# ch-andrei/VTAMIQ

Hardware: AMD Instinct MI355X
Metric: image-pairs/sec ViT-B/16 P=500 patches, 1->8 MI355X; % bf16 MFMA roofline (higher is better)
Workload: dtype f16

## Files before the change

### vtamiq_amd/csrc/cls_tail.hip

```cpp
#include <mutex>

#include "dev_common.h"
#include "kernels.h"

namespace vtq {
namespace {

template <int V4>
__global__ __launch_bounds__(256) void rows_ln_kernel(const float* __restrict__ src, int64_t stride, const float* __restrict__ w,
                                                      const float* __restrict__ b, float* __restrict__ ln, float* __restrict__ copy,
                                                      int rows, PlaneOut po, const int* __restrict__ vl_row0) {
    constexpr int H = 256 * V4;
    const int lane = threadIdx.x & 63;
    const int r = blockIdx.x * 4 + (threadIdx.x >> 6);
    if (r >= rows) return;
    const float4* xr = (const float4*)(src + (vl_row0 ? (int64_t)vl_row0[r] * H : r * stride));
    float4 v[V4];
    float s = 0.f;
#pragma unroll
    for (int i = 0; i < V4; ++i) {
        v[i] = xr[i * 64 + lane];
        if (copy) ((float4*)(copy + (int64_t)r * H))[i * 64 + lane] = v[i];
        s += (v[i].x + v[i].y) + (v[i].z + v[i].w);
    }
    const float mean = wave_sum(s) * (1.0f / H);
    float q = 0.f;
#pragma unroll
    for (int i = 0; i < V4; ++i) {
        v[i].x -= mean; v[i].y -= mean; v[i].z -= mean; v[i].w -= mean;
        q += (v[i].x * v[i].x + v[i].y * v[i].y) + (v[i].z * v[i].z + v[i].w * v[i].w);
    }
    const float rstd = 1.0f / sqrtf(wave_sum(q) * (1.0f / H) + 1e-6f);
#pragma unroll
    for (int i = 0; i < V4; ++i) {
        const float4 w4 = ((const float4*)w)[i * 64 + lane], b4 = ((const float4*)b)[i * 64 + lane];
        float4 y = {v[i].x * rstd * w4.x + b4.x, v[i].y * rstd * w4.y + b4.y, v[i].z * rstd * w4.z + b4.z, v[i].w * rstd * w4.w + b4.w};
        ((float4*)(ln + (int64_t)r * H))[i * 64 + lane] = y;
        plane_store4(po, r, (i * 64 + lane) * 4, y.x, y.y, y.z, y.w);
    }
}

constexpr int kFoldChunk = 64;
constexpr int kFoldSub = 32;
constexpr int kFoldPad = 16;

template <typename T, int WPL>
__global__ __launch_bounds__(1024) void cls_key_fold_kernel(const float* __restrict__ q, const T* __restrict__ wk, int64_t w_plane, int ldw,
                                                            float* __restrict__ u, int R, int H) {
    typedef typename Vec<T>::x4 tx4;
    __shared__ float qs[4][64];
    __shared__ __attribute__((aligned(16))) float red[3][4][1024];
    const int head = blockIdx.x, nh = gridDim.x, r0 = blockIdx.y * 4;
    const int ct = H >> 2, g = threadIdx.x / ct, c = 4 * (threadIdx.x - g * ct);
    const T* wr = wk + ((int64_t)head * 64 + g * 16) * ldw + c;
    tx4 wh[16], wl[16];
#pragma unroll
    for (int i = 0; i < 16; ++i) {
        wh[i] = *(const tx4*)(wr + (int64_t)i * ldw);
        if constexpr (WPL == 2) wl[i] = *(const tx4*)(wr + (int64_t)i * ldw + w_plane);
    }
    if (threadIdx.x < 256) {
        const int rr = threadIdx.x >> 6, d = threadIdx.x & 63;
        qs[rr][d] = (r0 + rr < R) ? q[(int64_t)(r0 + rr) * H + head * 64 + d] : 0.f;
    }
    __syncthreads();
    float acc[4][4];
#pragma unroll
    for (int rr = 0; rr < 4; ++rr)
#pragma unroll
        for (int e = 0; e < 4; ++e) acc[rr][e] = 0.f;
#pragma unroll
    for (int i = 0; i < 16; ++i) {
        float w[4];
#pragma unroll
        for (int e = 0; e < 4; ++e) {
            w[e] = (float)wh[i][e];
            if constexpr (WPL == 2) w[e] += (float)wl[i][e];
        }
#pragma unroll
        for (int rr = 0; rr < 4; ++rr) {
            const float qd = qs[rr][g * 16 + i];
#pragma unroll
            for (int e = 0; e < 4; ++e) acc[rr][e] = fmaf(qd, w[e], acc[rr][e]);
        }
    }
    if (g > 0) {
#pragma unroll
        for (int rr = 0; rr < 4; ++rr) *(float4*)&red[g - 1][rr][c] = float4{acc[rr][0], acc[rr][1], acc[rr][2], acc[rr][3]};
    }
    __syncthreads();
    if (g > 0) return;
#pragma unroll
    for (int rr = 0; rr < 4; ++rr) {
#pragma unroll
        for (int k = 0; k < 3; ++k) {
            const float4 o = *(const float4*)&red[k][rr][c];
            acc[rr][0] += o.x; acc[rr][1] += o.y; acc[rr][2] += o.z; acc[rr][3] += o.w;
        }
        if (r0 + rr < R) *(float4*)(u + ((int64_t)(r0 + rr) * nh + head) * H + c) = float4{acc[rr][0], acc[rr][1], acc[rr][2], acc[rr][3]};
    }
}

template <int V4>
__global__ __launch_bounds__(512) void cls_fold_attention_kernel(const float* __restrict__ x, int64_t seq_stride, const float* __restrict__ lw,
                                                                 const float* __restrict__ lb, const float* __restrict__ u,
                                                                 float* __restrict__ part, int S, int nh, int q_log2, VarSeq vl) {
    constexpr int H = 256 * V4, LD = H + kFoldPad, NG = 4 * V4, NB = 2 * V4;
    extern __shared__ __attribute__((aligned(16))) float fold_smem[];
    float* rows = fold_smem;
    float (*scp)[kFoldSub][16] = (float (*)[kFoldSub][16])(rows + kFoldSub * LD);
    float (*pr)[16] = (float (*)[16])(rows + kFoldSub * LD + 4 * kFoldSub * 16);
    float (*pp)[16] = (float (*)[16])(rows + kFoldSub * LD + 5 * kFoldSub * 16);
    float* run = rows + kFoldSub * LD + 6 * kFoldSub * 16;
    const int tid = threadIdx.x, lane = tid & 63, fr = lane & 15, fq = lane >> 4;
    const int wave = __builtin_amdgcn_readfirstlane(tid >> 6);
    const int chunk = blockIdx.x, seq = blockIdx.y, c0 = chunk * kFoldChunk;
    if (vl.len) {
        S = vl.len[seq];
        if (c0 >= S) return;
    }
    const float* xs = x + (vl.row0 ? (int64_t)vl.row0[seq] * H : (int64_t)seq * seq_stride);
    const int rb = wave & 1, kbase = (wave >> 1) * (H / 4);
    float4 uf[NG];
    {
        const float* ur = u + ((int64_t)seq * nh + (fr < nh ? fr : nh - 1)) * H + kbase + 4 * fq;
#pragma unroll
        for (int j = 0; j < NG; ++j) uf[j] = *(const float4*)(ur + 16 * j);
    }
    float4 v[4][V4];
    auto load_rows = [&](int sub) {
#pragma unroll
        for (int i = 0; i < 4; ++i) {
            const int srow = c0 + sub * kFoldSub + wave * 4 + i;
            if (srow < S) {
                const float4* xr = (const float4*)(xs + (int64_t)srow * H);
#pragma unroll
                for (int k = 0; k < V4; ++k) v[i][k] = xr[k * 64 + lane];
            } else {
#pragma unroll
                for (int k = 0; k < V4; ++k) v[i][k] = float4{0.f, 0.f, 0.f, 0.f};
            }
        }
    };
    f32x4 acc[NB];
#pragma unroll
    for (int b = 0; b < NB; ++b) acc[b] = f32x4{0.f, 0.f, 0.f, 0.f};
    f32x4 accl = {0.f, 0.f, 0.f, 0.f};
    if (tid < 16) run[tid] = -INFINITY;
    const int left = S - c0;
    const int nsub = left >= kFoldChunk ? kFoldChunk / kFoldSub : (left + kFoldSub - 1) / kFoldSub;
    load_rows(0);
    for (int sub = 0; sub < nsub; ++sub) {
        const int s0 = c0 + sub * kFoldSub;
        float4 w4[V4], b4[V4];
#pragma unroll
        for (int k = 0; k < V4; ++k) { w4[k] = ((const float4*)lw)[k * 64 + lane]; b4[k] = ((const float4*)lb)[k * 64 + lane]; }
#pragma unroll
        for (int i = 0; i < 4; ++i) {
            const int row = wave * 4 + i;
            const bool live = s0 + row < S;
            float s = 0.f;
#pragma unroll
            for (int k = 0; k < V4; ++k) s += (v[i][k].x + v[i][k].y) + (v[i][k].z + v[i][k].w);
            const float mean = wave_sum(s) * (1.0f / H);
            float qq = 0.f;
#pragma unroll
            for (int k = 0; k < V4; ++k) {
                v[i][k].x -= mean; v[i][k].y -= mean; v[i][k].z -= mean; v[i][k].w -= mean;
                qq += (v[i][k].x * v[i][k].x + v[i][k].y * v[i][k].y) + (v[i][k].z * v[i][k].z + v[i][k].w * v[i][k].w);
            }
            const float rstd = 1.0f / sqrtf(wave_sum(qq) * (1.0f / H) + 1e-6f);
#pragma unroll
            for (int k = 0; k < V4; ++k) {
                float4 y = {v[i][k].x * rstd * w4[k].x + b4[k].x, v[i][k].y * rstd * w4[k].y + b4[k].y, v[i][k].z * rstd * w4[k].z + b4[k].z,
                            v[i][k].w * rstd * w4[k].w + b4[k].w};
                if (!live) y = float4{0.f, 0.f, 0.f, 0.f};
                *(float4*)(rows + row * LD + (k * 64 + lane) * 4) = y;
            }
        }
        __syncthreads();
        if (sub + 1 < nsub) load_rows(sub + 1);
        {
            f32x4 sa = {0.f, 0.f, 0.f, 0.f}, sb = {0.f, 0.f, 0.f, 0.f};
            const float* ar = rows + (rb * 16 + fr) * LD + kbase + 4 * fq;
#pragma unroll
            for (int j = 0; j < NG; ++j) {
                const float4 a = *(const float4*)(ar + 16 * j);
                sa = __builtin_amdgcn_mfma_f32_16x16x4f32(a.x, uf[j].x, sa, 0, 0, 0);
                sb = __builtin_amdgcn_mfma_f32_16x16x4f32(a.y, uf[j].y, sb, 0, 0, 0);
                sa = __builtin_amdgcn_mfma_f32_16x16x4f32(a.z, uf[j].z, sa, 0, 0, 0);
                sb = __builtin_amdgcn_mfma_f32_16x16x4f32(a.w, uf[j].w, sb, 0, 0, 0);
            }
#pragma unroll
            for (int e = 0; e < 4; ++e) scp[wave >> 1][rb * 16 + 4 * fq + e][fr] = sa[e] + sb[e];
        }
        __syncthreads();
        const int row = tid >> 4, h = tid & 15;
        {
            float sc = (scp[0][row][h] + scp[1][row][h]) + (scp[2][row][h] + scp[3][row][h]);
            if (!q_log2) sc *= 0.125f;
            if (s0 + row >= S || h >= nh) sc = -INFINITY;
            pr[row][h] = sc;
        }
        __syncthreads();
        const float m_old = run[(sub & 1) * 16 + h];
        float mx = m_old;
#pragma unroll 8
        for (int r = 0; r < kFoldSub; ++r) mx = fmaxf(mx, pr[r][h]);
        {
            const float d = pr[row][h] - mx;
            pp[row][h] = h < nh ? (q_log2 ? exp2f(d) : expf(d)) : 0.f;
            if (tid < 16) {
                const float dm = m_old - mx;
                run[((sub + 1) & 1) * 16 + h] = mx;
                run[32 + h] = h < nh ? (q_log2 ? exp2f(dm) : expf(dm)) : 1.f;
            }
        }
        __syncthreads();
        {
            if (sub > 0) {
                const float4 al = *(const float4*)(run + 32 + 4 * fq);
#pragma unroll
                for (int b = 0; b < NB; ++b) { acc[b][0] *= al.x; acc[b][1] *= al.y; acc[b][2] *= al.z; acc[b][3] *= al.w; }
                accl[0] *= al.x; accl[1] *= al.y; accl[2] *= al.z; accl[3] *= al.w;
            }
            float pa[kFoldSub / 4];
#pragma unroll
            for (int s = 0; s < kFoldSub / 4; ++s) pa[s] = pp[4 * s + fq][fr];
#pragma unroll
            for (int s = 0; s < kFoldSub / 4; ++s) {
                const float* br = rows + (4 * s + fq) * LD + 16 * wave + fr;
#pragma unroll
                for (int b = 0; b < NB; ++b) acc[b] = __builtin_amdgcn_mfma_f32_16x16x4f32(pa[s], br[128 * b], acc[b], 0, 0, 0);
                if (wave == 0) accl = __builtin_amdgcn_mfma_f32_16x16x4f32(pa[s], 1.0f, accl, 0, 0, 0);
            }
        }
        __syncthreads();
    }
    float* pz = part + ((int64_t)seq * gridDim.x + chunk) * nh * (H + 2);
#pragma unroll
    for (int b = 0; b < NB; ++b)
#pragma unroll
        for (int e = 0; e < 4; ++e)
            if (4 * fq + e < nh) pz[(4 * fq + e) * H + 16 * wave + 128 * b + fr] = acc[b][e];
    if (tid < nh) pz[nh * H + 2 * tid] = run[(nsub & 1) * 16 + tid];
    if (wave == 0 && fr == 0) {
#pragma unroll
        for (int e = 0; e < 4; ++e)
            if (4 * fq + e < nh) pz[nh * H + 2 * (4 * fq + e) + 1] = accl[e];
    }
}

__global__ __launch_bounds__(256) void cls_fold_combine_kernel(const float* __restrict__ part, int nchunks, int H, PlaneOut po, int q_log2,
                                                               const int* __restrict__ vl_len) {
    const int head = blockIdx.x, nh = gridDim.x, seq = blockIdx.y, c4 = 4 * threadIdx.x;
    if (c4 >= H) return;
    const int64_t ps = (int64_t)nh * (H + 2);
    const float* pb = part + (int64_t)seq * nchunks * ps;
    if (vl_len) nchunks = (vl_len[seq] + kFoldChunk - 1) / kFoldChunk;
    const float* ml = pb + (int64_t)nh * H + 2 * head;
    float mx = -INFINITY;
    for (int c0 = 0; c0 < nchunks; c0 += 8) {
        float mv[8];
#pragma unroll
        for (int i = 0; i < 8; ++i) mv[i] = ml[(c0 + i < nchunks ? c0 + i : nchunks - 1) * ps];
#pragma unroll
        for (int i = 0; i < 8; ++i)
            if (c0 + i < nchunks) mx = fmaxf(mx, mv[i]);
    }
    float l = 0.f, z[4] = {0.f, 0.f, 0.f, 0.f};
    for (int c0 = 0; c0 < nchunks; c0 += 4) {
        float mv[4], lv[4];
        float4 zc[4];
#pragma unroll
        for (int i = 0; i < 4; ++i) {
            const int64_t o = (c0 + i < nchunks ? c0 + i : nchunks - 1) * ps;
            mv[i] = ml[o]; lv[i] = ml[o + 1];
            zc[i] = *(const float4*)(pb + o + (int64_t)head * H + c4);
        }
#pragma unroll
        for (int i = 0; i < 4; ++i) {
            if (c0 + i >= nchunks) break;
            const float d = mv[i] - mx;
            const float w = q_log2 ? exp2f(d) : expf(d);
            l = fmaf(w, lv[i], l);
            z[0] = fmaf(w, zc[i].x, z[0]); z[1] = fmaf(w, zc[i].y, z[1]); z[2] = fmaf(w, zc[i].z, z[2]); z[3] = fmaf(w, zc[i].w, z[3]);
        }
    }
    const float inv = 1.0f / l;
    plane_store4(po, seq, head * H + c4, z[0] * inv, z[1] * inv, z[2] * inv, z[3] * inv);
}

}

hipError_t launch_rows_ln(const float* src, int64_t stride, const float* w, const float* b, float* ln, float* copy, int rows, int H,
                          PlaneOut po, hipStream_t s, const int* vl_row0) {
    const dim3 g((rows + 3) / 4), blk(256);
    if (H == 768) hipLaunchKernelGGL(rows_ln_kernel<3>, g, blk, 0, s, src, stride, w, b, ln, copy, rows, po, vl_row0);
    else if (H == 1024) hipLaunchKernelGGL(rows_ln_kernel<4>, g, blk, 0, s, src, stride, w, b, ln, copy, rows, po, vl_row0);
    else return hipErrorInvalidValue;
    return hipGetLastError();
}

int cls_fold_chunk_rows() { return kFoldChunk; }

namespace {
template <int V4>
hipError_t launch_fold_attention(const float* x, int64_t seq_stride, const float* lw, const float* lb, const float* u, float* part, int nseq,
                                 int S, int nh, int q_log2, hipStream_t s, VarSeq vl) {
    constexpr int lds = (kFoldSub * (256 * V4 + kFoldPad) + 6 * kFoldSub * 16 + 48) * 4;
    {
        static std::mutex mu;
        static bool configured[64] = {false};
        int dev = 0;
        hipError_t e = hipGetDevice(&dev);
        if (e != hipSuccess) return e;
        std::lock_guard<std::mutex> lk(mu);
        if (dev < 0 || dev >= 64) return hipErrorInvalidDevice;
        if (!configured[dev]) {
            e = hipFuncSetAttribute((const void*)cls_fold_attention_kernel<V4>, hipFuncAttributeMaxDynamicSharedMemorySize, lds);
            if (e != hipSuccess) return e;
            configured[dev] = true;
        }
    }
    hipLaunchKernelGGL((cls_fold_attention_kernel<V4>), dim3((S + kFoldChunk - 1) / kFoldChunk, nseq), dim3(512), lds, s, x, seq_stride, lw, lb, u,
                       part, S, nh, q_log2, vl);
    return hipGetLastError();
}
}

hipError_t launch_cls_fold(const float* q, const void* wk, int64_t w_plane, int ldw, int f16_, int wplanes, const float* x, int64_t seq_stride,
                           const float* lw, const float* lb, float* u, float* part, int nseq, int S, int H, PlaneOut zo, hipStream_t s,
                           bool q_log2, VarSeq vl) {
    if ((vl.row0 != nullptr) != (vl.len != nullptr)) return hipErrorInvalidValue;
    if (nseq < 1 || S < 1 || (H != 768 && H != 1024) || ldw < H || ldw % 4 || (wplanes != 1 && wplanes != 2) || seq_stride % 4 || !zo.p || zo.ld < (H / 64) * H)
        return hipErrorInvalidValue;
    const int nh = H / 64, nchunks = (S + kFoldChunk - 1) / kFoldChunk;
    const dim3 gk(nh, (nseq + 3) / 4), blk(256);
#define VTQ_KF(TT, NP) hipLaunchKernelGGL((cls_key_fold_kernel<TT, NP>), gk, dim3(H), 0, s, q, (const TT*)wk, w_plane, ldw, u, nseq, H)
    if (!f16_) { if (wplanes == 1) VTQ_KF(bf16, 1); else VTQ_KF(bf16, 2); }
    else { if (wplanes == 1) VTQ_KF(f16, 1); else VTQ_KF(f16, 2); }
#undef VTQ_KF
    hipError_t e = hipGetLastError();
    if (e != hipSuccess) return e;
    e = H == 768 ? launch_fold_attention<3>(x, seq_stride, lw, lb, u, part, nseq, S, nh, q_log2 ? 1 : 0, s, vl)
                 : launch_fold_attention<4>(x, seq_stride, lw, lb, u, part, nseq, S, nh, q_log2 ? 1 : 0, s, vl);
    if (e != hipSuccess) return e;
    hipLaunchKernelGGL(cls_fold_combine_kernel, dim3(nh, nseq), blk, 0, s, (const float*)part, nchunks, H, zo, q_log2 ? 1 : 0, vl.len);
    return hipGetLastError();
}

}
```

Measured before the change: 2153.

## Batch several fold chunks per workgroup, swizzle LDS rows, use permlane max reduction

The CLS fold-attention kernel now has each workgroup process cpw consecutive 64-row chunks, with cpw chosen so about 256 workgroups launch in total. Partial outputs are still written per chunk, and the next tile's rows are prefetched across chunk boundaries. The LDS row layout is XOR-swizzled to reduce bank conflicts on the MFMA operand reads. The per-row score max now uses permlane16/32 swap reductions plus a small per-wave buffer instead of a 32-iteration LDS scan. The trade-off is fewer workgroups and less parallelism for small batches. The final load is clamped instead of branched, so it reads dummy rows.

```diff
diff --git a/vtamiq_amd/csrc/cls_tail.hip b/vtamiq_amd/csrc/cls_tail.hip
--- a/vtamiq_amd/csrc/cls_tail.hip
+++ b/vtamiq_amd/csrc/cls_tail.hip
@@ -1,3 +1,4 @@
+#include <algorithm>
 #include <mutex>
 
 #include "dev_common.h"
@@ -43,6 +44,23 @@
 constexpr int kFoldChunk = 64;
 constexpr int kFoldSub = 32;
 constexpr int kFoldPad = 16;
+constexpr int kFoldGroupWgs = 256;
+
+template <int M>
+__device__ __forceinline__ float fold_max_xor(float v) {
+    uint32_t a = __builtin_bit_cast(uint32_t, v), b = a;
+    asm volatile("" : "+v"(b));
+    uint32_t s0, s1;
+    if constexpr (M == 32) {
+        const auto sw = __builtin_amdgcn_permlane32_swap(a, b, false, false);
+        s0 = sw[0]; s1 = sw[1];
+    } else {
+        const auto sw = __builtin_amdgcn_permlane16_swap(a, b, false, false);
+        s0 = sw[0]; s1 = sw[1];
+    }
+    asm volatile("" : "+v"(s0), "+v"(s1));
+    return fmaxf(__builtin_bit_cast(float, s0), __builtin_bit_cast(float, s1));
+}
 
 template <typename T, int WPL>
 __global__ __launch_bounds__(1024) void cls_key_fold_kernel(const float* __restrict__ q, const T* __restrict__ wk, int64_t w_plane, int ldw,
@@ -104,21 +122,20 @@
 template <int V4>
 __global__ __launch_bounds__(512) void cls_fold_attention_kernel(const float* __restrict__ x, int64_t seq_stride, const float* __restrict__ lw,
                                                                  const float* __restrict__ lb, const float* __restrict__ u,
-                                                                 float* __restrict__ part, int S, int nh, int q_log2, VarSeq vl) {
+                                                                 float* __restrict__ part, int S, int nh, int q_log2, VarSeq vl, int nchunks,
+                                                                 int cpw) {
     constexpr int H = 256 * V4, LD = H + kFoldPad, NG = 4 * V4, NB = 2 * V4;
     extern __shared__ __attribute__((aligned(16))) float fold_smem[];
     float* rows = fold_smem;
     float (*scp)[kFoldSub][16] = (float (*)[kFoldSub][16])(rows + kFoldSub * LD);
-    float (*pr)[16] = (float (*)[16])(rows + kFoldSub * LD + 4 * kFoldSub * 16);
+    float* wm = rows + kFoldSub * LD + 4 * kFoldSub * 16;
     float (*pp)[16] = (float (*)[16])(rows + kFoldSub * LD + 5 * kFoldSub * 16);
     float* run = rows + kFoldSub * LD + 6 * kFoldSub * 16;
     const int tid = threadIdx.x, lane = tid & 63, fr = lane & 15, fq = lane >> 4;
     const int wave = __builtin_amdgcn_readfirstlane(tid >> 6);
-    const int chunk = blockIdx.x, seq = blockIdx.y, c0 = chunk * kFoldChunk;
-    if (vl.len) {
-        S = vl.len[seq];
-        if (c0 >= S) return;
-    }
+    const int cfirst = blockIdx.x * cpw, seq = blockIdx.y, r0 = cfirst * kFoldChunk;
+    if (vl.len) S = vl.len[seq];
+    if (r0 >= S) return;
     const float* xs = x + (vl.row0 ? (int64_t)vl.row0[seq] * H : (int64_t)seq * seq_stride);
     const int rb = wave & 1, kbase = (wave >> 1) * (H / 4);
     float4 uf[NG];
@@ -127,19 +144,16 @@
 #pragma unroll
         for (int j = 0; j < NG; ++j) uf[j] = *(const float4*)(ur + 16 * j);
     }
+    const int rend = min(S, r0 + cpw * kFoldChunk), nt = (rend - r0 + kFoldSub - 1) / kFoldSub;
     float4 v[4][V4];
-    auto load_rows = [&](int sub) {
+    auto load_rows = [&](int t) {
+        const int ln = t < nt ? lane : 0;
 #pragma unroll
         for (int i = 0; i < 4; ++i) {
-            const int srow = c0 + sub * kFoldSub + wave * 4 + i;
-            if (srow < S) {
-                const float4* xr = (const float4*)(xs + (int64_t)srow * H);
-#pragma unroll
-                for (int k = 0; k < V4; ++k) v[i][k] = xr[k * 64 + lane];
-            } else {
-#pragma unroll
-                for (int k = 0; k < V4; ++k) v[i][k] = float4{0.f, 0.f, 0.f, 0.f};
-            }
+            const int srow = min(r0 + t * kFoldSub + wave * 4 + i, rend - 1);
+            const float4* xr = (const float4*)(xs + (int64_t)srow * H);
+#pragma unroll
+            for (int k = 0; k < V4; ++k) v[i][k] = xr[k * 64 + ln];
         }
     };
     f32x4 acc[NB];
@@ -147,11 +161,9 @@
     for (int b = 0; b < NB; ++b) acc[b] = f32x4{0.f, 0.f, 0.f, 0.f};
     f32x4 accl = {0.f, 0.f, 0.f, 0.f};
     if (tid < 16) run[tid] = -INFINITY;
-    const int left = S - c0;
-    const int nsub = left >= kFoldChunk ? kFoldChunk / kFoldSub : (left + kFoldSub - 1) / kFoldSub;
     load_rows(0);
-    for (int sub = 0; sub < nsub; ++sub) {
-        const int s0 = c0 + sub * kFoldSub;
+    for (int t = 0; t < nt; ++t) {
+        const int sub = t & 1, s0 = r0 + t * kFoldSub;
         float4 w4[V4], b4[V4];
 #pragma unroll
         for (int k = 0; k < V4; ++k) { w4[k] = ((const float4*)lw)[k * 64 + lane]; b4[k] = ((const float4*)lb)[k * 64 + lane]; }
@@ -175,14 +187,14 @@
                 float4 y = {v[i][k].x * rstd * w4[k].x + b4[k].x, v[i][k].y * rstd * w4[k].y + b4[k].y, v[i][k].z * rstd * w4[k].z + b4[k].z,
                             v[i][k].w * rstd * w4[k].w + b4[k].w};
                 if (!live) y = float4{0.f, 0.f, 0.f, 0.f};
-                *(float4*)(rows + row * LD + (k * 64 + lane) * 4) = y;
-            }
-        }
-        __syncthreads();
-        if (sub + 1 < nsub) load_rows(sub + 1);
+                *(float4*)(rows + row * LD + (k * 64 + (lane ^ (wave & 3))) * 4) = y;
+            }
+        }
+        __syncthreads();
+        load_rows(t + 1);
         {
             f32x4 sa = {0.f, 0.f, 0.f, 0.f}, sb = {0.f, 0.f, 0.f, 0.f};
-            const float* ar = rows + (rb * 16 + fr) * LD + kbase + 4 * fq;
+            const float* ar = rows + (rb * 16 + fr) * LD + kbase + 4 * (fq ^ (fr >> 2));
 #pragma unroll
             for (int j = 0; j < NG; ++j) {
                 const float4 a = *(const float4*)(ar + 16 * j);
@@ -196,23 +208,27 @@
         }
         __syncthreads();
         const int row = tid >> 4, h = tid & 15;
-        {
-            float sc = (scp[0][row][h] + scp[1][row][h]) + (scp[2][row][h] + scp[3][row][h]);
-            if (!q_log2) sc *= 0.125f;
-            if (s0 + row >= S || h >= nh) sc = -INFINITY;
-            pr[row][h] = sc;
-        }
-        __syncthreads();
-        const float m_old = run[(sub & 1) * 16 + h];
-        float mx = m_old;
-#pragma unroll 8
-        for (int r = 0; r < kFoldSub; ++r) mx = fmaxf(mx, pr[r][h]);
-        {
-            const float d = pr[row][h] - mx;
+        float sc = (scp[0][row][h] + scp[1][row][h]) + (scp[2][row][h] + scp[3][row][h]);
+        if (!q_log2) sc *= 0.125f;
+        if (s0 + row >= S || h >= nh) sc = -INFINITY;
+        {
+            const float m4 = fold_max_xor<16>(fold_max_xor<32>(sc));
+            if (lane < 16) wm[h * 8 + wave] = m4;
+        }
+        __syncthreads();
+        const float m_old = run[sub * 16 + h];
+        float mx;
+        {
+            const float4 ma = *(const float4*)(wm + h * 8), mb = *(const float4*)(wm + h * 8 + 4);
+            mx = fmaxf(fmaxf(fmaxf(ma.x, ma.y), fmaxf(ma.z, ma.w)), fmaxf(fmaxf(mb.x, mb.y), fmaxf(mb.z, mb.w)));
+            mx = fmaxf(m_old, mx);
+        }
+        {
+            const float d = sc - mx;
             pp[row][h] = h < nh ? (q_log2 ? exp2f(d) : expf(d)) : 0.f;
             if (tid < 16) {
                 const float dm = m_old - mx;
-                run[((sub + 1) & 1) * 16 + h] = mx;
+                run[(sub ^ 1) * 16 + h] = mx;
                 run[32 + h] = h < nh ? (q_log2 ? exp2f(dm) : expf(dm)) : 1.f;
             }
         }
@@ -229,25 +245,31 @@
             for (int s = 0; s < kFoldSub / 4; ++s) pa[s] = pp[4 * s + fq][fr];
 #pragma unroll
             for (int s = 0; s < kFoldSub / 4; ++s) {
-                const float* br = rows + (4 * s + fq) * LD + 16 * wave + fr;
+                const float* br = rows + (4 * s + fq) * LD + 16 * wave + (fr ^ ((s & 3) << 2));
 #pragma unroll
                 for (int b = 0; b < NB; ++b) acc[b] = __builtin_amdgcn_mfma_f32_16x16x4f32(pa[s], br[128 * b], acc[b], 0, 0, 0);
                 if (wave == 0) accl = __builtin_amdgcn_mfma_f32_16x16x4f32(pa[s], 1.0f, accl, 0, 0, 0);
             }
         }
         __syncthreads();
-    }
-    float* pz = part + ((int64_t)seq * gridDim.x + chunk) * nh * (H + 2);
-#pragma unroll
-    for (int b = 0; b < NB; ++b)
-#pragma unroll
-        for (int e = 0; e < 4; ++e)
-            if (4 * fq + e < nh) pz[(4 * fq + e) * H + 16 * wave + 128 * b + fr] = acc[b][e];
-    if (tid < nh) pz[nh * H + 2 * tid] = run[(nsub & 1) * 16 + tid];
-    if (wave == 0 && fr == 0) {
-#pragma unroll
-        for (int e = 0; e < 4; ++e)
-            if (4 * fq + e < nh) pz[nh * H + 2 * (4 * fq + e) + 1] = accl[e];
+        if (sub == 1 || t + 1 == nt) {
+            float* pz = part + ((int64_t)seq * nchunks + cfirst + (t >> 1)) * nh * (H + 2);
+#pragma unroll
+            for (int b = 0; b < NB; ++b) {
+#pragma unroll
+                for (int e = 0; e < 4; ++e)
+                    if (4 * fq + e < nh) pz[(4 * fq + e) * H + 16 * wave + 128 * b + fr] = acc[b][e];
+                acc[b] = f32x4{0.f, 0.f, 0.f, 0.f};
+            }
+            if (tid < nh) pz[nh * H + 2 * tid] = run[(sub ^ 1) * 16 + tid];
+            if (wave == 0 && fr == 0) {
+#pragma unroll
+                for (int e = 0; e < 4; ++e)
+                    if (4 * fq + e < nh) pz[nh * H + 2 * (4 * fq + e) + 1] = accl[e];
+            }
+            accl = f32x4{0.f, 0.f, 0.f, 0.f};
+            if (tid < 16) run[tid] = -INFINITY;
+        }
     }
 }
 
@@ -323,8 +345,10 @@
             configured[dev] = true;
         }
     }
-    hipLaunchKernelGGL((cls_fold_attention_kernel<V4>), dim3((S + kFoldChunk - 1) / kFoldChunk, nseq), dim3(512), lds, s, x, seq_stride, lw, lb, u,
-                       part, S, nh, q_log2, vl);
+    const int nchunks = (S + kFoldChunk - 1) / kFoldChunk;
+    const int cpw = (int)std::min<int64_t>(nchunks, ((int64_t)nseq * nchunks + kFoldGroupWgs - 1) / kFoldGroupWgs);
+    hipLaunchKernelGGL((cls_fold_attention_kernel<V4>), dim3((nchunks + cpw - 1) / cpw, nseq), dim3(512), lds, s, x, seq_stride, lw, lb, u,
+                       part, S, nh, q_log2, vl, nchunks, cpw);
     return hipGetLastError();
 }
 }
```

After: 2155 (median of 6 runs). Within noise of the previous version (+0.1%).
